# ayutaz/F5-TTS

Measured on AMD Instinct MI355X. Metric: mel-frames/s (RTF alongside), F5TTS_v1_Base NFE=16 CFM.sample, higher is better.
Workload: dtype bf16; 1 GPU; C2: F5TTS_v1_Base CFM.sample, NFE 16 EPSS + sway -1, CFG 2.0, 1 utterance per GPU, 938 prompt + 938 generated frames (1876), 300 tokens; batch_per_gpu=1, frames=1876, gen_frames_per_gpu=938, nfe=16, parallelism=dp1

## Files before the change

f5-tts_amd/csrc/elementwise.hip:

```cpp
#include "common.h"
#include "kernels.h"
#include "lnrow.h"

#include <algorithm>

namespace f5h {

static inline unsigned nblk(int64_t n, int t) { return (unsigned)((n + t - 1) / t); }

struct TVals {
  float t[513];
};
__global__ void time_sinus_kernel(TVals tv, int n, float* out) {
  int i = blockIdx.x * blockDim.x + threadIdx.x;
  if (i >= n * 128) return;
  int r = i / 128, j = i % 128;
  const float k = logf(10000.f) / 127.f;
  float f = expf((float)j * -k);
  float e = (1000.f * tv.t[r]) * f;
  out[r * 256 + j] = sinf(e);
  out[r * 256 + 128 + j] = cosf(e);
}
hipError_t time_sinus(const float* t_host, int n, float* out, hipStream_t st) {
  if (n <= 0 || n > 512) return hipErrorInvalidValue;
// ... 690 lines not shown
  float v = 0.f;
  if (col < 128) {
    if (col < 100 && s < B && !drop_audio && cmask[(int64_t)b * N + n]) v = cond[((int64_t)b * N + n) * 100 + col];
  } else if (col - 128 < td) {
    const float* t = (s < B && !drop_text) ? tc : tu;
    v = t[((int64_t)b * N + n) * td + (col - 128)];
  }
  out[i] = from_f32<TO>(v);
}
hipError_t build_ct(int compute, const float* cond, const uint8_t* cond_mask, const float* text_c,
                    const float* text_u, int B, int N, int td, int S, int drop_audio, int drop_text, void* out,
                    hipStream_t st) {
  const int tdp = (td + 63) / 64 * 64;
  const int64_t total = (int64_t)S * N * (128 + tdp);
  F5H_OP_DISPATCH(compute, T, hipLaunchKernelGGL(build_ct_kernel<T>, dim3(nblk(total, 256)), dim3(256), 0, st, cond, cond_mask, text_c, text_u, B, N, td, tdp, S, drop_audio, drop_text, (T*)out););
  return hipGetLastError();
}

template <typename TO>
__global__ void pack_y_kernel(const float* y, int rows, int mel, TO* yp) {
  int64_t i = (int64_t)blockIdx.x * blockDim.x + threadIdx.x;
  if (i >= (int64_t)rows * 128) return;
  int64_t r = i >> 7;
  int c = (int)(i & 127);
  yp[i] = from_f32<TO>(c < mel ? y[r * mel + c] : 0.f);
}
hipError_t pack_y(int compute, const float* y, int rows, int mel, void* ypad, hipStream_t st) {
  const int64_t total = (int64_t)rows * 128;
  F5H_OP_DISPATCH(compute, T, hipLaunchKernelGGL(pack_y_kernel<T>, dim3(nblk(total, 256)), dim3(256), 0, st, y, rows, mel, (T*)ypad););
  return hipGetLastError();
}

template <typename TO>
__global__ __launch_bounds__(256) void cfg_euler_kernel(EulerArgs a, TO* ypad) {
  int64_t i = (int64_t)blockIdx.x * blockDim.x + threadIdx.x;
  const int64_t total = (int64_t)a.B * a.N * a.mel;
  const int k = a.kstep ? __hip_atomic_load(a.kstep, __ATOMIC_RELAXED, __HIP_MEMORY_SCOPE_AGENT) : 0;
  if (a.kstep && a.next_dst) {
    if (k + 1 < a.nfe) {
      const float4* src = reinterpret_cast<const float4*>(a.next_src + (int64_t)(k + 1) * a.next_stride);
      float4* dst = reinterpret_cast<float4*>(a.next_dst);
      for (int64_t j = i; j < a.next_n / 4; j += (int64_t)gridDim.x * blockDim.x) dst[j] = src[j];
    }
  }
  float dt = a.dt;
  float* traj = a.traj;
  if (a.kstep) {
    dt = sub_nc(a.tgrid[k + 1], a.tgrid[k]);
    traj = a.trajp ? *a.trajp : nullptr;
    if (traj) traj += (int64_t)(k + 1) * total;
  }
  for (; i < total; i += (int64_t)gridDim.x * blockDim.x) {
    const int c = (int)(i % a.mel);
    const int64_t bn = i / a.mel;
    const int b = (int)(bn / a.N), n = (int)(bn - (int64_t)b * a.N);
    const float pc = a.p[(int64_t)b * a.p_seq_stride + (int64_t)(a.p_row_off + n) * a.p_ld + c];
    float v = pc;
    if (a.use_cfg) {
      const float pu = a.p[(int64_t)(a.B + b) * a.p_seq_stride + (int64_t)(a.p_row_off + n) * a.p_ld + c];
      v = add_nc(pc, mul_nc(sub_nc(pc, pu), a.cfg));
    }
    const float y = add_nc(a.y[i], mul_nc(dt, v));
    a.y[i] = y;
    if (ypad) ypad[bn * 128 + c] = from_f32<TO>(y);
    if (traj) traj[i] = y;
  }
  if (a.kstep && a.arrive) {
    __syncthreads();
    if (threadIdx.x == 0) {
      const unsigned old = __hip_atomic_fetch_add(a.arrive, 1u, __ATOMIC_RELAXED, __HIP_MEMORY_SCOPE_AGENT);
      if (old == gridDim.x - 1) {
        __hip_atomic_store(a.arrive, 0u, __ATOMIC_RELAXED, __HIP_MEMORY_SCOPE_AGENT);
        __hip_atomic_store(const_cast<int*>(a.kstep), k + 1, __ATOMIC_RELAXED, __HIP_MEMORY_SCOPE_AGENT);
        if (a.tick) __hip_atomic_fetch_add(a.tick, 1, __ATOMIC_RELAXED, __HIP_MEMORY_SCOPE_AGENT);
      }
    }
  }
}
hipError_t cfg_euler(const EulerArgs& a, hipStream_t st) {
  const int64_t total = (int64_t)a.B * a.N * a.mel;
  const unsigned blocks = std::min<unsigned>(128, std::max<unsigned>(1, nblk(total, 256)));
  F5H_OP_DISPATCH(a.compute, T, hipLaunchKernelGGL(cfg_euler_kernel<T>, dim3(blocks), dim3(256), 0, st, a, (T*)a.ypad););
  return hipGetLastError();
}

template <typename TO, int METHOD>
__global__ __launch_bounds__(256) void cfg_rk_kernel(RkArgs a, TO* ypad) {
  constexpr OdeTableau T = ode_tableau(METHOD);
  constexpr int STAGES = T.stages;
  static_assert(METHOD == 1 || METHOD == 2, "midpoint or rk4");
  static_assert(METHOD != 1 || (T.a[4] == T.c[1] && T.b[0] == 0.f && T.b[1] == 1.f), "midpoint tableau");
  static_assert(METHOD != 2 || (T.a[4] == T.c[1] && T.a[8] == -T.c[1] && T.a[9] == 1.f && T.a[12] == 1.f &&
                                T.a[13] == -1.f && T.a[14] == 1.f && T.b[1] == 3.f * T.b[0] &&
                                T.b[2] == T.b[1] && T.b[3] == T.b[0]),
                "3/8-rule tableau");
  int64_t i = (int64_t)blockIdx.x * blockDim.x + threadIdx.x;
  const int64_t total = (int64_t)a.B * a.N * a.mel;
  const int e = __hip_atomic_load(a.keval, __ATOMIC_RELAXED, __HIP_MEMORY_SCOPE_AGENT);
  const int k = e / STAGES, s = e - k * STAGES;
  if (a.next_dst && e + 1 < a.neval) {
    const float4* src = reinterpret_cast<const float4*>(a.next_src + (int64_t)(e + 1) * a.next_stride);
    float4* dst = reinterpret_cast<float4*>(a.next_dst);
    for (int64_t j = i; j < a.next_n / 4; j += (int64_t)gridDim.x * blockDim.x) dst[j] = src[j];
  }
  const float dt = sub_nc(a.sgrid[k + 1], a.sgrid[k]);
  const bool last = s == STAGES - 1;
  float* traj = (last && a.trajp) ? *a.trajp : nullptr;
  if (traj) traj += (int64_t)(k + 1) * total;
  for (; i < total; i += (int64_t)gridDim.x * blockDim.x) {
    const int c = (int)(i % a.mel);
    const int64_t bn = i / a.mel;
    const int b = (int)(bn / a.N), n = (int)(bn - (int64_t)b * a.N);
    const float pc = a.p[(int64_t)b * a.p_seq_stride + (int64_t)(a.p_row_off + n) * a.p_ld + c];
    float v = pc;
    if (a.use_cfg) {
// ... 221 lines not shown
```

f5-tts_amd/csrc/engine_ctl.cpp:

```cpp
#include "engine_internal.h"
#include "capi_util.h"

thread_local std::string g_err;
int fail(int code, const std::string& msg) {
  g_err = msg;
  return code;
}
int f5h_internal_fail(int code, const std::string& msg) { return fail(code, msg); }

extern "C" {

const char* f5h_last_error(void) { return g_err.c_str(); }
const char* f5h_version(void) { return "f5h 0.1 gfx950"; }

int f5h_probe_enable(f5h_engine* e, int32_t kclass, int32_t enable) {
  if (!e) return fail(F5H_EINVAL, "null engine");
  std::lock_guard<std::mutex> g(e->pm);
  e->probe_class = enable ? kclass : -1;
  if (e->pstamp) {
    HIPCK(hipSetDevice(e->dev));
    HIPCK(hipDeviceSynchronize());
    HIPCK(hipMemset(e->pstamp, 0, 64 * sizeof(unsigned long long)));
    HIPCK(hipMemset(e->pslots, 0xff, (size_t)kProbeEnd * sizeof(unsigned long long)));
    HIPCK(hipMemset(e->pslots + kProbeEnd, 0, (size_t)kProbeEnd * sizeof(unsigned long long)));
// ... 119 lines not shown
    if (e->mx8_count) {
      HIPCK(hipSetDevice(e->dev));
      HIPCK(hipMemcpy(&n, e->mx8_count, sizeof(n), hipMemcpyDeviceToHost));
    }
    *launches = (int64_t)n;
  }
  return 0;
}

int f5h_store_policy_force(int32_t mode) {
  if (mode < -1 || mode > 1) return fail(F5H_EINVAL, "forced store policy must be -1 (off), 0 (plain) or 1 (write-through)");
  store_policy_force(mode);
  g_kernel_epoch.fetch_add(1);
  return 0;
}

int f5h_last_call_host_ms(f5h_engine* e, double* ms, int32_t n) {
  if (!e || !ms || n <= 0) return fail(F5H_EINVAL, "null engine / buffer");
  std::lock_guard<std::mutex> g(e->hm);
  for (int i = 0; i < n; ++i) ms[i] = i < kHostPhases ? e->last_host[i] : 0.0;
  return 0;
}

int f5h_graph_stats(f5h_engine* e, int64_t* captures, int64_t* replays, int32_t* cached) {
  if (!e) return fail(F5H_EINVAL, "null engine");
  std::lock_guard<std::mutex> g(e->gm);
  if (captures) *captures = e->n_captures;
  if (replays) *replays = e->n_replays;
  if (cached) *cached = (int32_t)e->graphs.size();
  return 0;
}

int f5h_gemm_force_config(int32_t cfg) {
  if (cfg != -1 && cfg != 0 && cfg != 1 && cfg != 5 && cfg != 11 && cfg != 12 && cfg != 13)
    return fail(F5H_EINVAL, "gemm config must be -1, 0, 1, 5, 11, 12 or 13");
  gemm_force_config(cfg);
  g_kernel_epoch.fetch_add(1);
  return 0;
}

int f5h_attn_force_safe(int32_t on) {
  attention_force_safe(on);
  g_kernel_epoch.fetch_add(1);
  return 0;
}

}
```

f5-tts_amd/csrc/gemm.hip:

```cpp
#include "gemm_impl.h"

namespace f5h {

static int g_force_cfg = -1;
static int gemm_env_cfg() {
  static int v = [] {
    const char* e = getenv("F5H_GEMM_CFG");
    return e ? atoi(e) : -1;
  }();
  return v;
}


static int large_cfg() {
  static const int v = [] {
    const char* e = getenv("F5H_LARGE_CFG");
    const int c = e ? atoi(e) : 11;
    return (c == 12 || c == 13) ? c : 11;
  }();
  return v;
}

int gemm_group_m() {
  static const int v = [] {
    const char* e = getenv("F5H_GEMM_GROUP_M");
    const int g = e ? atoi(e) : 1;
    return g > 1 && g <= 64 ? g : 1;
  }();
  return v;
}

int gemm_num_cus() {
  static int cus[64] = {0};
  int dev = 0;
  if (hipGetDevice(&dev) != hipSuccess || dev < 0 || dev >= 64) return 256;
  if (!cus[dev]) {
    int n = 0;
    if (hipDeviceGetAttribute(&n, hipDeviceAttributeMultiprocessorCount, dev) != hipSuccess || n <= 0) n = 256;
    cus[dev] = n;
  }
  return cus[dev];
}

static int pick_cfg(const GemmArgs& a) {
  if (a.K % 64 == 0 && (int64_t)((a.M + 255) / 256) * ((a.N + 255) / 256) >= 1024) return large_cfg();
  struct Opt { int cfg, bm, bn; float eff; };
  constexpr Opt opts[3] = {{5, 192, 128, 0.86f}, {1, 128, 128, 0.74f}, {0, 64, 128, 0.57f}};
  int best = 0;
  double tbest = 1e300;
  for (const Opt& o : opts) {
    const int64_t tiles = (int64_t)((a.M + o.bm - 1) / o.bm) * ((a.N + o.bn - 1) / o.bn);
    const double t = (double)((tiles + 511) / 512) * o.bm * o.bn / o.eff;
    if (t < tbest * 0.999) tbest = t, best = o.cfg;
  }
  return best;
}

static int gemm_map_cfg(int N, int K) {
  struct E { int n, k, c; };
  static std::vector<E> m = [] {
    std::vector<E> v;
    const char* e = getenv("F5H_GEMM_MAP");
    while (e && *e) {
      int n, k, c, used = 0;
      if (sscanf(e, "%d:%d:%d%n", &n, &k, &c, &used) != 3) break;
      v.push_back({n, k, c});
      e += used;
      if (*e == ',') ++e;
    }
    return v;
  }();
  for (const E& x : m)
    if (x.n == N && x.k == K) return x.c;
  return -1;
}


int gemm_select_cfg(const GemmArgs& a) {
  int cfg = g_force_cfg >= 0 ? g_force_cfg : gemm_env_cfg();
  if (cfg < 0) cfg = gemm_map_cfg(a.N, a.K);
  if (cfg < 0) cfg = pick_cfg(a);
  return cfg;
}

hipError_t gemm_launch_bf16_a(int epi, const GemmArgs& a, hipStream_t st);
hipError_t gemm_launch_bf16_b(int epi, const GemmArgs& a, hipStream_t st);
hipError_t gemm_launch_f16_a(int epi, const GemmArgs& a, hipStream_t st);
hipError_t gemm_launch_f16_b(int epi, const GemmArgs& a, hipStream_t st);
hipError_t gemm_launch_f32(int epi, const GemmArgs& a, hipStream_t st);

static bool hot_epi(int epi) {
  return epi == EPI_QKV || epi == EPI_RESID || epi == EPI_RESID16 || epi == EPI_GELU_TANH || epi == EPI_GELU_ERF_OP;
}

void gemm_force_config(int cfg) { g_force_cfg = cfg; }

static int g_store_force = -1;
void store_policy_force(int mode) { g_store_force = mode; }
int store_policy_forced() { return g_store_force; }

static bool gemm_wt_variant(int compute, int epi, const GemmArgs& a, int64_t* tiles, int64_t* slots) {
  if (compute == F5H_C_FP32 || (epi != EPI_QKV && epi != EPI_RESID16 && epi != EPI_GELU_TANH) || a.M <= 0) return false;
  const int cfg = gemm_select_cfg(a);
  if (cfg != 0 && cfg != 1 && cfg != 5) return false;
  const int bm = cfg == 0 ? 64 : (cfg == 1 ? 128 : 192);
  *tiles = (int64_t)((a.M + bm - 1) / bm) * ((a.N + 127) / 128);
  *slots = 2 * (int64_t)gemm_num_cus();
  return epi == EPI_QKV ? fast_epi_ok<EPI_QKV>(a, 128)
                        : (epi == EPI_RESID16 ? fast_epi_ok<EPI_RESID16>(a, 128) : fast_epi_ok<EPI_GELU_TANH>(a, 128));
}

int gemm_store_wt(int compute, int epi, const GemmArgs& a, int want) {
  if (g_store_force >= 0) want = g_store_force;
  int64_t tiles = 0, slots = 0;
  if (want == 0 || !gemm_wt_variant(compute, epi, a, &tiles, &slots)) return 0;
  return want > 0 || tiles <= slots;
}

hipError_t gemm(int compute, int epi, const GemmArgs& a0, hipStream_t st) {
  GemmArgs a = a0;
  if (g_store_force >= 0) a.store_wt = gemm_store_wt(compute, epi, a0, g_store_force);
  const int bke = compute ? 64 : 32;
  if (a.K % bke != 0 || a.M < 0 || a.N <= 0 || a.lda % 8 || a.ldw % 8) return hipErrorInvalidValue;
  if (epi == EPI_INPROJ && (a.ldc % 8 || a.ld_add % 8 || a.N % 8)) return hipErrorInvalidValue;
  if (epi == EPI_QKV && (a.N % 64)) return hipErrorInvalidValue;
  if (a.A2 && (a.k_split <= 0 || a.k_split % 64 || a.k_split >= a.K)) return hipErrorInvalidValue;
  if (a.resid && epi != EPI_RESID && epi != EPI_RESID16) return hipErrorInvalidValue;
  switch (compute) {
    case F5H_C_BF16: return hot_epi(epi) ? gemm_launch_bf16_a(epi, a, st) : gemm_launch_bf16_b(epi, a, st);
    case F5H_C_FP16: return hot_epi(epi) ? gemm_launch_f16_a(epi, a, st) : gemm_launch_f16_b(epi, a, st);
    default: return gemm_launch_f32(epi, a, st);
  }
}

}
```

f5-tts_amd/csrc/gemm_impl.h:

```cpp
#pragma once
#include "common.h"
#include "kernels.h"
#include "chain.h"

#include <cstdio>
#include <cstdlib>
#include <vector>

namespace f5h {

int gemm_select_cfg(const GemmArgs& a);


template <int BM, int BN, int WGM, int WGN, int NS, int KB = 128>
struct GemmCfg {
  static constexpr int NW = WGM * WGN, THREADS = 64 * NW;
  static constexpr int WM = BM / WGM, WN = BN / WGN, MT = WM / 16, NT = WN / 16;
  static constexpr int CPR = KB / 16;
  static constexpr int stage_bytes = (BM + BN) * KB;
  static constexpr int main_bytes = NS * stage_bytes;
  static constexpr int EPAD = WN + 4;
  static constexpr int epi_bytes = NW * 16 * EPAD * 4;
  static constexpr int bytes = main_bytes > epi_bytes ? main_bytes : epi_bytes;
  static_assert(KB == 128 || KB == 64, "stage row bytes");
// ... 206 lines not shown
        if (col + e < g.N) C[off + e] = x.v[e];
    }
  }
}

template <int DPS, int X = 0>
F5H_DEV void wait_stages(int n_stages) {
  switch (n_stages) {
    case 0: asm volatile("s_waitcnt vmcnt(%0)" ::"i"(X) : "memory"); break;
    case 1: asm volatile("s_waitcnt vmcnt(%0)" ::"i"(DPS + X) : "memory"); break;
    case 2: asm volatile("s_waitcnt vmcnt(%0)" ::"i"(2 * DPS + X) : "memory"); break;
    case 3: asm volatile("s_waitcnt vmcnt(%0)" ::"i"(3 * DPS + X) : "memory"); break;
    default: asm volatile("s_waitcnt vmcnt(%0)" ::"i"(4 * DPS + X) : "memory"); break;
  }
}

template <int AUX = 0>
F5H_DEV void store16_rs(__amdgpu_buffer_rsrc_t r, uint32_t off, u32x4 v) {
  __builtin_amdgcn_raw_buffer_store_b128(v, r, off, 0, AUX);
}
template <typename TC, int AUX = 0>
F5H_DEV void store8_rs(__amdgpu_buffer_rsrc_t r, uint32_t elem, const V8& x) {
  if constexpr (is16<TC>()) {
    typedef typename Op16<TC>::v8 v8;
    const v8 b = {from_f32<TC>(x.v[0]), from_f32<TC>(x.v[1]), from_f32<TC>(x.v[2]), from_f32<TC>(x.v[3]),
                  from_f32<TC>(x.v[4]), from_f32<TC>(x.v[5]), from_f32<TC>(x.v[6]), from_f32<TC>(x.v[7])};
    store16_rs<AUX>(r, elem * 2u, __builtin_bit_cast(u32x4, b));
  } else {
    store16_rs<AUX>(r, elem * 4u, u32x4{__float_as_uint(x.v[0]), __float_as_uint(x.v[1]), __float_as_uint(x.v[2]),
                                   __float_as_uint(x.v[3])});
    store16_rs<AUX>(r, elem * 4u + 16u, u32x4{__float_as_uint(x.v[4]), __float_as_uint(x.v[5]), __float_as_uint(x.v[6]),
                                         __float_as_uint(x.v[7])});
  }
}

typedef unsigned u32x2_t __attribute__((ext_vector_type(2)));
template <int CTRL>
F5H_DEV float dpp8(float x) {
  return __int_as_float(__builtin_amdgcn_update_dpp(0, __float_as_int(x), CTRL, 0xF, 0xF, false));
}
F5H_DEV float sum8(float v) {
  v = add_nc(v, dpp8<0xB1>(v));
  v = add_nc(v, dpp8<0x4E>(v));
  return add_nc(v, dpp8<0x141>(v));
}
F5H_DEV V8 qk_norm8(V8 x, const V8& w, float eps, bool on) {
  float s = mul_nc(x.v[0], x.v[0]);
#pragma unroll
  for (int e = 1; e < 8; ++e) s = add_nc(s, mul_nc(x.v[e], x.v[e]));
  const float r = rsqrtf(add_nc(mul_nc(sum8(s), 1.f / 64.f), eps));
#pragma unroll
  for (int e = 0; e < 8; ++e) x.v[e] = on ? mul_nc(mul_nc(x.v[e], r), w.v[e]) : x.v[e];
  return x;
}
F5H_DEV float ln_m2_term(float q, float mp, float mean) {
  const float d = sub_nc(mp, mean);
  return __builtin_fmaf(mul_nc(64.f, d), d, q);
}
F5H_DEV float ln_rstd(float m2, float inv_np, float eps) {
  return rsqrtf(__builtin_fmaf(m2, mul_nc(inv_np, 1.f / 64.f), eps));
}
F5H_DEV float sum8_order(const float (&a)[8]) {
  return add_nc(add_nc(add_nc(a[0], a[1]), add_nc(a[2], a[3])), add_nc(add_nc(a[4], a[5]), add_nc(a[6], a[7])));
}
F5H_DEV void ln_row_fetch(const GemmArgs& g, int m0, int tid, int BM, u32x4 (&raw)[8]) {
  const bool on = g.ln_part_in != nullptr;
// ... 36 lines not shown
  const int cc = lane % CH;
  const int col = cbase + cc * 8;
  V8 bias8 = V8{};
  if constexpr (BIAS) bias8 = load8(g.bias + col);
  V8 lnA = V8{}, lnB = V8{};
  __amdgpu_buffer_rsrc_t ln_dst = rsrc_of(nullptr, 0), ln_st = rsrc_of(nullptr, 0);
  int ln_p = 0;
  const int ln_np = g.ln_nparts;
  if constexpr (LNF == 1 || LNF == 4) {
    if constexpr (LNF == 1) {
      lnA = load8(g.hs_scale + col);
#pragma unroll
      for (int e = 0; e < 8; ++e) lnA.v[e] = 1.f + lnA.v[e];
      ln_dst = rsrc_of(g.hs, (uint64_t)g.M * g.ldc * sizeof(TC));
    }
    ln_st = rsrc_of(g.ln_part, (uint64_t)g.M * ln_np * 8);
    ln_p = __builtin_amdgcn_readfirstlane(cbase >> 6);
  } else if constexpr (LNCONS) {
    if (g.ln_u) lnA = load8(g.ln_u + col);
    if (g.ln_v) lnB = load8(g.ln_v + col);
    if constexpr (BIAS) {
#pragma unroll
      for (int e = 0; e < 8; ++e) lnB.v[e] += bias8.v[e];
    }
    if constexpr (LNF == 2) ln_st = rsrc_of(g.ln_part_in, (uint64_t)g.M * ln_np * 8);
  }
  const int lp0 = min(cc, ln_np - 1), lp1 = min(cc + 8, ln_np - 1);
  const float ln_w0 = cc < ln_np ? 1.f : 0.f, ln_w1 = cc + 8 < ln_np ? 1.f : 0.f;
  const float ln_inv_np = 1.f / (float)ln_np;
  V8 gate8 = V8{{1.f, 1.f, 1.f, 1.f, 1.f, 1.f, 1.f, 1.f}};
  if constexpr (EPI == EPI_RESID || EPI == EPI_RESID16)
    if (g.gate) gate8 = load8(g.gate + col);
  int which = 0, head = 0, dh = 0;
  bool rope_on = false;
  float qsc = 1.f;
  __amdgpu_buffer_rsrc_t dst;
  if constexpr (EPI == EPI_QKV) {
    static_assert(WN <= 64 && 64 % WN == 0, "a wave's columns lie in one head");
    const int inner = g.heads * 64;
    which = __builtin_amdgcn_readfirstlane(fdiv(cbase, inner));
    const int hc = col - which * inner;
    head = hc >> 6;
    dh = hc & 63;
    rope_on = which < 2 && head < g.rope_heads;
    qsc = (which == 0 && g.q_scale != 0.f) ? g.q_scale : 1.f;
    dst = rsrc_of(which == 0 ? g.q : (which == 1 ? g.k : g.v), qkv_dst_elems(g, g.qkv_dst_len ? fdiv(g.M, g.seq_len) : 0) * sizeof(TC));
  } else {
    constexpr int OES = (EPI == EPI_STORE || EPI == EPI_RESID || EPI == EPI_INPROJ) ? 4 : (int)sizeof(TC);
    dst = rsrc_of(g.C, (uint64_t)(g.M + (EPI == EPI_INPROJ ? g.dual_rows : 0)) * g.ldc * OES);
  }
  const int dlen = EPI == EPI_QKV ? qkv_panel_rows(g) : 0;
  V8 qkw = V8{};
  if constexpr (QKN) qkw = load8((which == 0 ? g.q_norm_w : g.k_norm_w) + dh);
  const bool qkn_on = which < 2;
  struct RowIn {
    u32x4 d0, d1;
    u32x4 e0, e1;
    uint32_t kb;
    u32x2_t s0, s1;
  };
  const __amdgpu_buffer_rsrc_t rk = rsrc_of(g.rowkeep, g.rowkeep ? (uint64_t)g.M : 0);
  const bool masked = g.rowkeep != nullptr;
  int pf_sq[TPC], pf_pos[TPC], ps_sq[TPC], ps_pos[TPC];
  if constexpr (EPI == EPI_QKV) {
#pragma unroll
    for (int t = 0; t < TPC; ++t) {
      const int row0 = rbase + t * (64 / CH) + lane / CH;
      pf_sq[t] = ps_sq[t] = fdiv(row0, g.seq_len);
      pf_pos[t] = ps_pos[t] = row0 - pf_sq[t] * g.seq_len;
    }
  }
  auto advance = [&](int& sq, int& pos) {
    pos += 16;
    while (pos >= g.seq_len) {
      pos -= g.seq_len;
      ++sq;
    }
  };
  auto fetch = [&](int i, RowIn (&ri)[TPC]) {
#pragma unroll
    for (int t = 0; t < TPC; ++t) {
      const int rr = t * (64 / CH) + lane / CH;
      const int rowc = min(rbase + i * 16 + rr, g.M - 1);
      if constexpr (LNF == 2) {
        ri[t].s0 = __builtin_amdgcn_raw_buffer_load_b64(ln_st, (uint32_t)((rowc * ln_np + lp0) * 8), 0, 0);
        ri[t].s1 = __builtin_amdgcn_raw_buffer_load_b64(ln_st, (uint32_t)((rowc * ln_np + lp1) * 8), 0, 0);
      }
      if constexpr (EPI == EPI_QKV) {
        (void)rowc;
        const u32x4* p = reinterpret_cast<const u32x4*>(g.rope + pf_pos[t] * 32 + (dh >> 1));
        ri[t].d0 = p[0];
        ri[t].d1 = p[1];
        advance(pf_sq[t], pf_pos[t]);
      } else if constexpr (EPI == EPI_RESID || EPI == EPI_RESID16) {
        if constexpr (!PREF) {
          const u32x4* p = reinterpret_cast<const u32x4*>(reinterpret_cast<const ResT<TC, EPI>*>(
                                                              g.resid ? g.resid : g.C) + (int64_t)rowc * g.ldc + col);
          ri[t].d0 = p[0];
          if constexpr (sizeof(ResT<TC, EPI>) == 4) ri[t].d1 = p[1];
        }
        ri[t].kb = __builtin_amdgcn_raw_buffer_load_b8(rk, (uint32_t)rowc, 0, 0);
      } else if constexpr (EPI == EPI_INPROJ) {
        const u32x4* p = reinterpret_cast<const u32x4*>(g.add + (int64_t)rowc * g.ld_add + col);
        ri[t].d0 = p[0];
        ri[t].d1 = p[1];
        const u32x4* p2 = reinterpret_cast<const u32x4*>(g.add + (int64_t)(rowc + g.dual_rows) * g.ld_add + col);
        ri[t].e0 = p2[0];
        ri[t].e1 = p2[1];
      }
    }
  };
  auto as_v8 = [&](const RowIn& ri) -> V8 {
    if constexpr (EPI == EPI_RESID16 && is16<TC>()) {
      typedef typename Op16<TC>::v8 v8;
      const v8 h = __builtin_bit_cast(v8, ri.d0);
      return V8{{to_f32(h[0]), to_f32(h[1]), to_f32(h[2]), to_f32(h[3]), to_f32(h[4]), to_f32(h[5]), to_f32(h[6]),
                 to_f32(h[7])}};
    } else {
      return V8{{__uint_as_float(ri.d0[0]), __uint_as_float(ri.d0[1]), __uint_as_float(ri.d0[2]),
                 __uint_as_float(ri.d0[3]), __uint_as_float(ri.d1[0]), __uint_as_float(ri.d1[1]),
                 __uint_as_float(ri.d1[2]), __uint_as_float(ri.d1[3])}};
    }
  };
  constexpr int RB = PD + 1;
  RowIn rbuf[RB][TPC];
  static_for<0, (PD < MT ? PD : MT)>([&](auto F) { fetch(decltype(F)::value, rbuf[decltype(F)::value % RB]); });
  static_for<0, MT>([&](auto I) {
    constexpr int i = decltype(I)::value;
    if constexpr (i + PD < MT) fetch(i + PD, rbuf[(i + PD) % RB]);
#pragma unroll
    for (int j = 0; j < NT; ++j)
      *reinterpret_cast<f32x4*>(Cs + fr * EPAD + j * 16 + 4 * q) = acc[i][j];
    __builtin_amdgcn_fence(__ATOMIC_RELEASE, "wavefront");
    __builtin_amdgcn_wave_barrier();
    __builtin_amdgcn_fence(__ATOMIC_ACQUIRE, "wavefront");
#pragma unroll
    for (int t = 0; t < TPC; ++t) {
      const int rr = t * (64 / CH) + lane / CH;
      const int row = rbase + i * 16 + rr;
      const float* src = Cs + rr * EPAD + cc * 8;
      const float4 a0 = *reinterpret_cast<const float4*>(src), a1 = *reinterpret_cast<const float4*>(src + 4);
      V8 x{{a0.x, a0.y, a0.z, a0.w, a1.x, a1.y, a1.z, a1.w}};
      const RowIn& ri = rbuf[i % RB][t];
      if constexpr (LNCONS) {
        float m, rstd;
        if constexpr (LNF == 3) {
          const float2 ms = *reinterpret_cast<const float2*>(ln_rows + 2 * (i * 16 + rr));
          m = ms.x;
          rstd = ms.y;
        } else {
        const float m0 = __uint_as_float(ri.s0.x), m1 = __uint_as_float(ri.s1.x);
        m = mul_nc(sum8(add_nc(ln_w0 * m0, ln_w1 * m1)), ln_inv_np);
        const float e0 = ln_m2_term(__uint_as_float(ri.s0.y), m0, m), e1 = ln_m2_term(__uint_as_float(ri.s1.y), m1, m);
        rstd = ln_rstd(sum8(add_nc(ln_w0 * e0, ln_w1 * e1)), ln_inv_np, g.ln_eps);
        }
#pragma unroll
        for (int e = 0; e < 8; e += 2) {
          const f32x2 t = f32x2{x.v[e], x.v[e + 1]} - f32x2{m, m} * f32x2{lnA.v[e], lnA.v[e + 1]};
          const f32x2 y = f32x2{rstd, rstd} * t + f32x2{lnB.v[e], lnB.v[e + 1]};
          x.v[e] = y.x;
          x.v[e + 1] = y.y;
        }
      }
      if constexpr (BIAS && !LNCONS) {
#pragma unroll
        for (int e = 0; e < 8; ++e) x.v[e] = add_nc(x.v[e], bias8.v[e]);
      }
      if constexpr (QKN) x = qk_norm8(x, qkw, g.qk_norm_eps, qkn_on);
      if constexpr (EPI == EPI_QKV) {
        const V8 cs = as_v8(ri);
#pragma unroll
        for (int p = 0; p < 4; ++p) {
          const float c = cs.v[2 * p], sn = cs.v[2 * p + 1];
          const f32x2 ab = {x.v[2 * p], x.v[2 * p + 1]};
          f32x2 r;
          {
#pragma clang fp contract(off)
            const f32x2 pc = ab * c, ps = f32x2{ab.y, ab.x} * sn;
            r = pc + f32x2{-ps.x, ps.y};
            r = (rope_on ? r : ab) * qsc;
          }
          x.v[2 * p] = r.x;
          x.v[2 * p + 1] = r.y;
        }
        (void)row;
        store8_rs<TC, AUX>(dst, (uint32_t)(((ps_sq[t] * g.heads + head) * dlen + ps_pos[t]) * 64 + dh), x);
        advance(ps_sq[t], ps_pos[t]);
      } else if constexpr (EPI == EPI_RESID || EPI == EPI_RESID16) {
        V8 c;
        if constexpr (PREF)
          c = pre[PREF ? i : 0][PREF ? t : 0];
        else
          c = as_v8(ri);
        const bool keep = !masked || ri.kb;
        V8 o;
#pragma unroll
        for (int e = 0; e < 8; ++e) o.v[e] = resid_add(c.v[e], gate8.v[e], x.v[e], keep);
        store8_rs<ResT<TC, EPI>, AUX>(dst, (uint32_t)((int64_t)row * g.ldc + col), o);
        if constexpr (LNF == 1 || LNF == 4) {
          V8 hr, hv;
          f32x2 s2 = {0.f, 0.f};
#pragma unroll
          for (int e = 0; e < 8; e += 2) {
            const f32x2 h2 = {to_f32(from_f32<TC>(o.v[e])), to_f32(from_f32<TC>(o.v[e + 1]))};
            hr.v[e] = h2.x;
            hr.v[e + 1] = h2.y;
            if constexpr (LNF == 1) {
              const f32x2 v2 = h2 * f32x2{lnA.v[e], lnA.v[e + 1]};
              hv.v[e] = v2.x;
              hv.v[e + 1] = v2.y;
              s2 += h2;
            }
          }
          if constexpr (LNF == 1) store8_rs<TC, AUX>(ln_dst, (uint32_t)((int64_t)row * g.ldc + col), hv);
          const float mean = LNF == 4 ? 0.f : sum8(s2.x + s2.y) * (1.f / 64.f);
          f32x2 q2 = {0.f, 0.f};
#pragma unroll
          for (int e = 0; e < 8; e += 2) {
            const f32x2 dv = f32x2{hr.v[e], hr.v[e + 1]} - f32x2{mean, mean};
            q2 += dv * dv;
          }
          const float m2 = sum8(q2.x + q2.y);
          __builtin_amdgcn_raw_buffer_store_b64(u32x2_t{__float_as_uint(mean), __float_as_uint(m2)}, ln_st,
                                                (uint32_t)((row * ln_np + ln_p) * 8), 0, 0);
        }
      } else if constexpr (EPI == EPI_GELU_TANH || EPI == EPI_GELU_ERF_OP) {
        if constexpr (EPI == EPI_GELU_TANH && is16<TC>()) {
#pragma unroll
          for (int e = 0; e < 8; e += 2) {
            const f32x2 gv = gelu_tanh_fast2(f32x2{x.v[e], x.v[e + 1]});
            x.v[e] = gv.x;
            x.v[e + 1] = gv.y;
          }
        } else {
#pragma unroll
          for (int e = 0; e < 8; ++e) x.v[e] = EPI == EPI_GELU_ERF_OP ? gelu_erf(x.v[e]) : gelu_tanh(x.v[e]);
        }
        store8_rs<TC, AUX>(dst, (uint32_t)((int64_t)row * g.ldc + col), x);
      } else if constexpr (EPI == EPI_STORE16) {
        store8_rs<TC, AUX>(dst, (uint32_t)((int64_t)row * g.ldc + col), x);
      } else if constexpr (EPI == EPI_INPROJ) {
        V8 o0, o1;
#pragma unroll
        for (int e = 0; e < 4; ++e) {
          o0.v[e] = x.v[e] + __uint_as_float(ri.d0[e]);
          o0.v[e + 4] = x.v[e + 4] + __uint_as_float(ri.d1[e]);
          o1.v[e] = x.v[e] + __uint_as_float(ri.e0[e]);
          o1.v[e + 4] = x.v[e + 4] + __uint_as_float(ri.e1[e]);
        }
        constexpr uint32_t kPast = 0xF0000000u / 4;
        store8_rs<float, AUX>(dst, row < g.M ? (uint32_t)((int64_t)row * g.ldc + col) : kPast, o0);
        if (g.dual_rows)
          store8_rs<float, AUX>(dst, row < g.M ? (uint32_t)((int64_t)(row + g.dual_rows) * g.ldc + col) : kPast, o1);
      } else {
        store8_rs<float, AUX>(dst, (uint32_t)((int64_t)row * g.ldc + col), x);
      }
    }
    __builtin_amdgcn_fence(__ATOMIC_RELEASE, "wavefront");
    __builtin_amdgcn_wave_barrier();
    __builtin_amdgcn_fence(__ATOMIC_ACQUIRE, "wavefront");
  });
}
template <typename TC, int EPI, int MT, int NT, int WN, int EPAD, bool PREF, int AUX = 0, int PD = 1, bool FOLD = true,
          bool QKN = false, int PM, int PT>
F5H_DEV void epilogue_fast(const GemmArgs& g, const f32x4 (&acc)[MT][NT], float* Cs, int rbase, int cbase,
                           int lane, const V8 (&pre)[PM][PT], const float* ln_rows = nullptr) {
  if constexpr (WN == 64 && is16<TC>() && FOLD) {
    if constexpr (EPI == EPI_RESID16) {
      if (g.ln_part && g.ln_rms) {
        if (g.bias)
          epilogue_fast_t<TC, EPI, MT, NT, WN, EPAD, PREF, true, PM, PT, AUX, PD, 4>(g, acc, Cs, rbase, cbase, lane, pre);
        else
          epilogue_fast_t<TC, EPI, MT, NT, WN, EPAD, PREF, false, PM, PT, AUX, PD, 4>(g, acc, Cs, rbase, cbase, lane, pre);
        return;
      }
      if (g.ln_part) {
        if (g.bias)
          epilogue_fast_t<TC, EPI, MT, NT, WN, EPAD, PREF, true, PM, PT, AUX, PD, 1>(g, acc, Cs, rbase, cbase, lane, pre);
        else
          epilogue_fast_t<TC, EPI, MT, NT, WN, EPAD, PREF, false, PM, PT, AUX, PD, 1>(g, acc, Cs, rbase, cbase, lane, pre);
        return;
      }
    } else if constexpr (EPI == EPI_GELU_TANH || EPI == EPI_QKV) {
      if (g.ln_part_in && ln_rows) {
        if (g.bias)
          epilogue_fast_t<TC, EPI, MT, NT, WN, EPAD, PREF, true, PM, PT, AUX, PD, 3, QKN>(g, acc, Cs, rbase, cbase, lane, pre,
                                                                                   ln_rows);
        else
          epilogue_fast_t<TC, EPI, MT, NT, WN, EPAD, PREF, false, PM, PT, AUX, PD, 3, QKN>(g, acc, Cs, rbase, cbase, lane, pre,
                                                                                    ln_rows);
        return;
      }
      if (g.ln_part_in) {
        if (g.bias)
// ... 1168 lines not shown
  if (a.q_norm_w)
    hipLaunchKernelGGL((gemm_kernel<TC, EPI_QKV, BM, 128, 2, 2, NS, false, 128, 0, true, true>), dim3(tiles), dim3(256), 0,
                       st, a);
  else
    hipLaunchKernelGGL((gemm_kernel<TC, EPI_QKV, BM, 128, 2, 2, NS, false, 128, 0, false, true>), dim3(tiles), dim3(256),
                       0, st, a);
  return hipGetLastError();
}

template <typename TC, int EPI>
static hipError_t launch_t(const GemmArgs& a, hipStream_t st) {
  if (a.M == 0) return hipSuccess;
  if constexpr (EPI == EPI_QKV) {
    if (a.add) {
      const bool qkn = a.q_norm_w || a.k_norm_w;
      if (a.ln_part_in || a.qkv_dst_len <= 0 || a.heads <= 0 || a.N != 3 * a.heads * 64 ||
          (qkn && (!a.q_norm_w || !a.k_norm_w)))
        return hipErrorInvalidValue;
      if constexpr (std::is_same<TC, bf16>::value) return gemm_launch_rq_bf16(a, st);
      else if constexpr (std::is_same<TC, float>::value) return gemm_launch_rq_f32(a, st);
      else return gemm_launch_rq_f16(a, st);
    }
  }
  int cfg = 0;
  if constexpr (is16<TC>()) cfg = gemm_select_cfg(a);
  const bool qkn = a.q_norm_w || a.k_norm_w;
  if (qkn && (EPI != EPI_QKV || !a.q_norm_w || !a.k_norm_w || a.heads <= 0 || a.N != 3 * a.heads * 64))
    return hipErrorInvalidValue;
  if (a.qkv_dst_len) {
    if (EPI != EPI_QKV || a.ln_part_in || a.seq_len <= 0 || a.qkv_dst_len < a.seq_len || a.M % a.seq_len ||
        a.M >= (1 << 24) || a.heads <= 0 || qkv_dst_elems(a, a.M / a.seq_len) * 4 >= 0xF0000000ull)
      return hipErrorInvalidValue;
  }
  const bool strips = a.ln_part || a.ln_part_in || qkn;
  if (strips && (cfg == 12 || cfg == 13)) cfg = 11;
  if (strips && cfg == 11 && (!fast_epi_ok<EPI>(a, 256) || a.K % 64)) cfg = 1;
  if (a.hs || a.ln_part || a.ln_part_in) {
    const bool prod = a.ln_part && EPI == EPI_RESID16 && (a.ln_rms ? !a.hs && !a.hs_scale : a.hs && a.hs_scale);
    const bool cons = a.ln_part_in && (EPI == EPI_GELU_TANH || EPI == EPI_QKV) &&
                      (a.ln_rms ? !a.ln_u && !a.ln_v : a.ln_u && a.ln_v);
    const int bn = cfg == 11 ? 256 : 128;
    if (!is16<TC>() || (a.ln_part && a.ln_part_in) || !(prod || cons) || a.ln_nparts <= 0 || a.ln_nparts > 16 ||
        (cfg != 0 && cfg != 1 && cfg != 5 && cfg != 11) || !fast_epi_ok<EPI>(a, bn) || (a.rowkeep && !a.ln_rms) ||
        a.live_len)
      return hipErrorInvalidValue;
  }
  if constexpr (EPI == EPI_QKV) {
    if (qkn) {
      if (cfg != 0 && cfg != 1 && cfg != 5 && cfg != 11) return hipErrorInvalidValue;
      if constexpr (std::is_same<TC, bf16>::value) return gemm_launch_qkn_bf16(a, cfg, st);
      else if constexpr (std::is_same<TC, float>::value) return gemm_launch_qkn_f32(a, cfg, st);
      else return gemm_launch_qkn_f16(a, cfg, st);
    }
  }
  switch (cfg) {
    case 0: return launch_cfg<TC, EPI, 64, 128, 2, 2, 3>(a, st);
    case 1: return launch_cfg<TC, EPI, 128, 128, 2, 2, 2>(a, st);
    case 5: return launch_cfg<TC, EPI, 192, 128, 2, 2, 2>(a, st);
    default:
      if constexpr (is16<TC>()) {
        if (a.K % 64) return hipErrorInvalidValue;
        if (cfg != 11 && cfg != 12 && cfg != 13) return hipErrorInvalidValue;
        if (cfg == 11)
          launch_pp<TC, EPI, 256, 256, 1, 4, 1, 3>(a, st);
        else if (cfg == 13)
          launch_ppp<TC, EPI, 256, 256, 1, 4, 1, 3>(a, st);
        else
          launch_8p<TC, EPI>(a, st);
        break;
      }
      return hipErrorInvalidValue;
  }
  return hipGetLastError();
}

template <typename TC>
static hipError_t launch_epi(int epi, const GemmArgs& a, hipStream_t st) {
  switch (epi) {
    case EPI_STORE: return launch_t<TC, EPI_STORE>(a, st);
    case EPI_SILU: return launch_t<TC, EPI_SILU>(a, st);
    case EPI_GELU_TANH: return launch_t<TC, EPI_GELU_TANH>(a, st);
    case EPI_GELU_ERF: return launch_t<TC, EPI_GELU_ERF>(a, st);
    case EPI_RESID: return launch_t<TC, EPI_RESID>(a, st);
    case EPI_RESID16: return launch_t<TC, EPI_RESID16>(a, st);
    case EPI_RESID_FILL: return launch_t<TC, EPI_RESID_FILL>(a, st);
    case EPI_INPROJ: return launch_t<TC, EPI_INPROJ>(a, st);
    case EPI_QKV: return launch_t<TC, EPI_QKV>(a, st);
    case EPI_GELU_ERF_OP: return launch_t<TC, EPI_GELU_ERF_OP>(a, st);
    case EPI_STORE16: return launch_t<TC, EPI_STORE16>(a, st);
  }
// ... 6 lines not shown
```

Before: 20220 mel-frames/s.

## Add small-tile GEMM config for narrow outputs and vectorize CFG Euler step

Adds a new GEMM config 2 (32x64 tiles, 6 stages) that the picker selects when N<=128 and the small-tile grid fits within the CU count. This targets narrow projections such as the mel output head, where 64x128 tiles leave most CUs idle. The config is limited to the plain-store epilogue and falls back to config 0 elsewhere. The CFG Euler update kernel now uses float4 loads and stores when alignment allows, runs 512 threads per block, and moves the next-row copy after the main loop (prefetching the first element) to cut scalar memory traffic and overlap the copy.

```diff
diff --git a/f5-tts_amd/csrc/elementwise.hip b/f5-tts_amd/csrc/elementwise.hip
--- a/f5-tts_amd/csrc/elementwise.hip
+++ b/f5-tts_amd/csrc/elementwise.hip
@@ -746,17 +746,28 @@
 }
 
 template <typename TO>
-__global__ __launch_bounds__(256) void cfg_euler_kernel(EulerArgs a, TO* ypad) {
-  int64_t i = (int64_t)blockIdx.x * blockDim.x + threadIdx.x;
+F5H_DEV void store_row4(TO* p, float x, float y, float z, float w) {
+  if constexpr (sizeof(TO) == 4) {
+    *reinterpret_cast<float4*>(p) = make_float4(x, y, z, w);
+  } else {
+    struct alignas(8) Q { TO v[4]; };
+    *reinterpret_cast<Q*>(p) = Q{{from_f32<TO>(x), from_f32<TO>(y), from_f32<TO>(z), from_f32<TO>(w)}};
+  }
+}
+
+template <typename TO, bool V4>
+__global__ __launch_bounds__(512) void cfg_euler_kernel(EulerArgs a, TO* ypad) {
+  const int64_t tid = (int64_t)blockIdx.x * blockDim.x + threadIdx.x, nthr = (int64_t)gridDim.x * blockDim.x;
   const int64_t total = (int64_t)a.B * a.N * a.mel;
   const int k = a.kstep ? __hip_atomic_load(a.kstep, __ATOMIC_RELAXED, __HIP_MEMORY_SCOPE_AGENT) : 0;
-  if (a.kstep && a.next_dst) {
-    if (k + 1 < a.nfe) {
-      const float4* src = reinterpret_cast<const float4*>(a.next_src + (int64_t)(k + 1) * a.next_stride);
-      float4* dst = reinterpret_cast<float4*>(a.next_dst);
-      for (int64_t j = i; j < a.next_n / 4; j += (int64_t)gridDim.x * blockDim.x) dst[j] = src[j];
-    }
-  }
+  const bool copy_row = a.kstep && a.next_dst && k + 1 < a.nfe;
+  const float4* const row_src =
+      copy_row ? reinterpret_cast<const float4*>(a.next_src + (int64_t)(k + 1) * a.next_stride) : nullptr;
+  float4* const row_dst = reinterpret_cast<float4*>(a.next_dst);
+  const int64_t row_n4 = a.next_n / 4;
+  const bool row_first = copy_row && tid < row_n4;
+  float4 row0 = make_float4(0.f, 0.f, 0.f, 0.f);
+  if (row_first) row0 = row_src[tid];
   float dt = a.dt;
   float* traj = a.traj;
   if (a.kstep) {
@@ -764,21 +775,58 @@
     traj = a.trajp ? *a.trajp : nullptr;
     if (traj) traj += (int64_t)(k + 1) * total;
   }
-  for (; i < total; i += (int64_t)gridDim.x * blockDim.x) {
-    const int c = (int)(i % a.mel);
-    const int64_t bn = i / a.mel;
-    const int b = (int)(bn / a.N), n = (int)(bn - (int64_t)b * a.N);
-    const float pc = a.p[(int64_t)b * a.p_seq_stride + (int64_t)(a.p_row_off + n) * a.p_ld + c];
-    float v = pc;
-    if (a.use_cfg) {
-      const float pu = a.p[(int64_t)(a.B + b) * a.p_seq_stride + (int64_t)(a.p_row_off + n) * a.p_ld + c];
-      v = add_nc(pc, mul_nc(sub_nc(pc, pu), a.cfg));
-    }
-    const float y = add_nc(a.y[i], mul_nc(dt, v));
-    a.y[i] = y;
-    if (ypad) ypad[bn * 128 + c] = from_f32<TO>(y);
-    if (traj) traj[i] = y;
-  }
+  if constexpr (V4) {
+    const int m4 = a.mel >> 2;
+    const bool traj4 = (reinterpret_cast<uintptr_t>(traj) & 15) == 0;
+    for (int64_t j = tid; j < total / 4; j += nthr) {
+      const int64_t bn = j / m4;
+      const int c = (int)(j - bn * m4) * 4;
+      const int b = (int)(bn / a.N), n = (int)(bn - (int64_t)b * a.N);
+      const float* pr = a.p + (int64_t)b * a.p_seq_stride + (int64_t)(a.p_row_off + n) * a.p_ld + c;
+      const float4 pc = *reinterpret_cast<const float4*>(pr);
+      float4 v = pc;
+      if (a.use_cfg) {
+        const float4 pu = *reinterpret_cast<const float4*>(pr + (int64_t)a.B * a.p_seq_stride);
+        v.x = add_nc(pc.x, mul_nc(sub_nc(pc.x, pu.x), a.cfg));
+        v.y = add_nc(pc.y, mul_nc(sub_nc(pc.y, pu.y), a.cfg));
+        v.z = add_nc(pc.z, mul_nc(sub_nc(pc.z, pu.z), a.cfg));
+        v.w = add_nc(pc.w, mul_nc(sub_nc(pc.w, pu.w), a.cfg));
+      }
+      float4 y = reinterpret_cast<const float4*>(a.y)[j];
+      y.x = add_nc(y.x, mul_nc(dt, v.x));
+      y.y = add_nc(y.y, mul_nc(dt, v.y));
+      y.z = add_nc(y.z, mul_nc(dt, v.z));
+      y.w = add_nc(y.w, mul_nc(dt, v.w));
+      reinterpret_cast<float4*>(a.y)[j] = y;
+      if (ypad) store_row4<TO>(ypad + bn * 128 + c, y.x, y.y, y.z, y.w);
+      if (traj) {
+        if (traj4) {
+          reinterpret_cast<float4*>(traj)[j] = y;
+        } else {
+          traj[4 * j] = y.x, traj[4 * j + 1] = y.y, traj[4 * j + 2] = y.z, traj[4 * j + 3] = y.w;
+        }
+      }
+    }
+  } else {
+    for (int64_t i = tid; i < total; i += nthr) {
+      const int c = (int)(i % a.mel);
+      const int64_t bn = i / a.mel;
+      const int b = (int)(bn / a.N), n = (int)(bn - (int64_t)b * a.N);
+      const float pc = a.p[(int64_t)b * a.p_seq_stride + (int64_t)(a.p_row_off + n) * a.p_ld + c];
+      float v = pc;
+      if (a.use_cfg) {
+        const float pu = a.p[(int64_t)(a.B + b) * a.p_seq_stride + (int64_t)(a.p_row_off + n) * a.p_ld + c];
+        v = add_nc(pc, mul_nc(sub_nc(pc, pu), a.cfg));
+      }
+      const float y = add_nc(a.y[i], mul_nc(dt, v));
+      a.y[i] = y;
+      if (ypad) ypad[bn * 128 + c] = from_f32<TO>(y);
+      if (traj) traj[i] = y;
+    }
+  }
+  if (row_first) row_dst[tid] = row0;
+  if (copy_row)
+    for (int64_t j = tid + nthr; j < row_n4; j += nthr) row_dst[j] = row_src[j];
   if (a.kstep && a.arrive) {
     __syncthreads();
     if (threadIdx.x == 0) {
@@ -793,8 +841,15 @@
 }
 hipError_t cfg_euler(const EulerArgs& a, hipStream_t st) {
   const int64_t total = (int64_t)a.B * a.N * a.mel;
-  const unsigned blocks = std::min<unsigned>(128, std::max<unsigned>(1, nblk(total, 256)));
-  F5H_OP_DISPATCH(a.compute, T, hipLaunchKernelGGL(cfg_euler_kernel<T>, dim3(blocks), dim3(256), 0, st, a, (T*)a.ypad););
+  auto al16 = [](const void* p) { return (reinterpret_cast<uintptr_t>(p) & 15) == 0; };
+  const bool v4 = a.mel % 4 == 0 && a.p_ld % 4 == 0 && a.p_seq_stride % 4 == 0 && al16(a.y) && al16(a.p) &&
+                  al16(a.ypad) && al16(a.traj);
+  const unsigned blocks = std::min<unsigned>(128, std::max<unsigned>(1, nblk(v4 ? total / 4 : total, 512)));
+  if (v4) {
+    F5H_OP_DISPATCH(a.compute, T, hipLaunchKernelGGL((cfg_euler_kernel<T, true>), dim3(blocks), dim3(512), 0, st, a, (T*)a.ypad););
+  } else {
+    F5H_OP_DISPATCH(a.compute, T, hipLaunchKernelGGL((cfg_euler_kernel<T, false>), dim3(blocks), dim3(512), 0, st, a, (T*)a.ypad););
+  }
   return hipGetLastError();
 }
 
diff --git a/f5-tts_amd/csrc/engine_ctl.cpp b/f5-tts_amd/csrc/engine_ctl.cpp
--- a/f5-tts_amd/csrc/engine_ctl.cpp
+++ b/f5-tts_amd/csrc/engine_ctl.cpp
@@ -175,8 +175,8 @@
 }
 
 int f5h_gemm_force_config(int32_t cfg) {
-  if (cfg != -1 && cfg != 0 && cfg != 1 && cfg != 5 && cfg != 11 && cfg != 12 && cfg != 13)
-    return fail(F5H_EINVAL, "gemm config must be -1, 0, 1, 5, 11, 12 or 13");
+  if (cfg != -1 && cfg != 0 && cfg != 1 && cfg != 2 && cfg != 5 && cfg != 11 && cfg != 12 && cfg != 13)
+    return fail(F5H_EINVAL, "gemm config must be -1, 0, 1, 2, 5, 11, 12 or 13");
   gemm_force_config(cfg);
   g_kernel_epoch.fetch_add(1);
   return 0;
diff --git a/f5-tts_amd/csrc/gemm.hip b/f5-tts_amd/csrc/gemm.hip
--- a/f5-tts_amd/csrc/gemm.hip
+++ b/f5-tts_amd/csrc/gemm.hip
@@ -44,6 +44,7 @@
 
 static int pick_cfg(const GemmArgs& a) {
   if (a.K % 64 == 0 && (int64_t)((a.M + 255) / 256) * ((a.N + 255) / 256) >= 1024) return large_cfg();
+  if (a.N <= 128 && (int64_t)((a.M + 31) / 32) * ((a.N + 63) / 64) <= gemm_num_cus()) return 2;
   struct Opt { int cfg, bm, bn; float eff; };
   constexpr Opt opts[3] = {{5, 192, 128, 0.86f}, {1, 128, 128, 0.74f}, {0, 64, 128, 0.57f}};
   int best = 0;
@@ -101,7 +102,8 @@
 
 static bool gemm_wt_variant(int compute, int epi, const GemmArgs& a, int64_t* tiles, int64_t* slots) {
   if (compute == F5H_C_FP32 || (epi != EPI_QKV && epi != EPI_RESID16 && epi != EPI_GELU_TANH) || a.M <= 0) return false;
-  const int cfg = gemm_select_cfg(a);
+  int cfg = gemm_select_cfg(a);
+  if (cfg == 2) cfg = 0;
   if (cfg != 0 && cfg != 1 && cfg != 5) return false;
   const int bm = cfg == 0 ? 64 : (cfg == 1 ? 128 : 192);
   *tiles = (int64_t)((a.M + bm - 1) / bm) * ((a.N + 127) / 128);
diff --git a/f5-tts_amd/csrc/gemm_impl.h b/f5-tts_amd/csrc/gemm_impl.h
--- a/f5-tts_amd/csrc/gemm_impl.h
+++ b/f5-tts_amd/csrc/gemm_impl.h
@@ -1826,6 +1826,7 @@
         a.M >= (1 << 24) || a.heads <= 0 || qkv_dst_elems(a, a.M / a.seq_len) * 4 >= 0xF0000000ull)
       return hipErrorInvalidValue;
   }
+  if (cfg == 2 && EPI != EPI_STORE) cfg = 0;
   const bool strips = a.ln_part || a.ln_part_in || qkn;
   if (strips && (cfg == 12 || cfg == 13)) cfg = 11;
   if (strips && cfg == 11 && (!fast_epi_ok<EPI>(a, 256) || a.K % 64)) cfg = 1;
@@ -1850,6 +1851,9 @@
   switch (cfg) {
     case 0: return launch_cfg<TC, EPI, 64, 128, 2, 2, 3>(a, st);
     case 1: return launch_cfg<TC, EPI, 128, 128, 2, 2, 2>(a, st);
+    case 2:
+      if constexpr (is16<TC>() && EPI == EPI_STORE) return launch_cfg<TC, EPI, 32, 64, 2, 2, 6>(a, st);
+      return hipErrorInvalidValue;
     case 5: return launch_cfg<TC, EPI, 192, 128, 2, 2, 2>(a, st);
     default:
       if constexpr (is16<TC>()) {
```

Result: no change. 20260 mel-frames/s (median of 4 runs) (+0.2%).

## Specialize GEMM epilogue on rope/scale/mask flags and strength-reduce QKV addressing

Applied to the files above, without the earlier changes.

Wraps the fast epilogue strip loop in a lambda instantiated per runtime-uniform form (rope on/off, q scaling on/off, row mask on/off). Unused rope-table loads, rowkeep byte loads and select logic are dropped on paths that do not need them. The per-row sequence/position division loop is replaced by an incremental offset with a precomputed wrap delta. Rope, bias and residual math now use packed f32x2 ops via inline asm, and the LN path reuses the packed bf16 output. Code size and register pressure grow from the multiple instantiations, and the inline asm may constrain scheduling.

```diff
diff --git a/f5-tts_amd/csrc/gemm_impl.h b/f5-tts_amd/csrc/gemm_impl.h
--- a/f5-tts_amd/csrc/gemm_impl.h
+++ b/f5-tts_amd/csrc/gemm_impl.h
@@ -262,6 +262,25 @@
     store16_rs<AUX>(r, elem * 4u + 16u, u32x4{__float_as_uint(x.v[4]), __float_as_uint(x.v[5]), __float_as_uint(x.v[6]),
                                          __float_as_uint(x.v[7])});
   }
+}
+
+template <typename TC>
+F5H_DEV uint32_t pack2(f32x2 v) {
+  typedef TC v2 __attribute__((ext_vector_type(2)));
+  return __builtin_bit_cast(uint32_t, v2{from_f32<TC>(v.x), from_f32<TC>(v.y)});
+}
+template <typename TC>
+F5H_DEV f32x2 unpack2(uint32_t w) {
+  typedef TC v2 __attribute__((ext_vector_type(2)));
+  const v2 h = __builtin_bit_cast(v2, w);
+  return f32x2{to_f32(h[0]), to_f32(h[1])};
+}
+F5H_DEV f32x2 rope_pair(f32x2 ab, f32x2 cs) {
+  f32x2 pc, ps, r;
+  asm("v_pk_mul_f32 %0, %1, %2 op_sel_hi:[1,0]" : "=v"(pc) : "v"(ab), "v"(cs));
+  asm("v_pk_mul_f32 %0, %1, %2 op_sel:[1,1] op_sel_hi:[0,1]" : "=v"(ps) : "v"(ab), "v"(cs));
+  asm("v_pk_add_f32 %0, %1, %2 neg_lo:[0,1]" : "=v"(r) : "v"(pc), "v"(ps));
+  return r;
 }
 
 typedef unsigned u32x2_t __attribute__((ext_vector_type(2)));
@@ -364,18 +383,13 @@
   if constexpr (EPI == EPI_RESID || EPI == EPI_RESID16)
     if (g.gate) gate8 = load8(g.gate + col);
   int which = 0, head = 0, dh = 0;
-  bool rope_on = false;
-  float qsc = 1.f;
   __amdgpu_buffer_rsrc_t dst;
   if constexpr (EPI == EPI_QKV) {
     static_assert(WN <= 64 && 64 % WN == 0, "a wave's columns lie in one head");
     const int inner = g.heads * 64;
     which = __builtin_amdgcn_readfirstlane(fdiv(cbase, inner));
-    const int hc = col - which * inner;
-    head = hc >> 6;
-    dh = hc & 63;
-    rope_on = which < 2 && head < g.rope_heads;
-    qsc = (which == 0 && g.q_scale != 0.f) ? g.q_scale : 1.f;
+    head = __builtin_amdgcn_readfirstlane((cbase - which * inner) >> 6);
+    dh = col & 63;
     dst = rsrc_of(which == 0 ? g.q : (which == 1 ? g.k : g.v), qkv_dst_elems(g, g.qkv_dst_len ? fdiv(g.M, g.seq_len) : 0) * sizeof(TC));
   } else {
     constexpr int OES = (EPI == EPI_STORE || EPI == EPI_RESID || EPI == EPI_INPROJ) ? 4 : (int)sizeof(TC);
@@ -393,23 +407,33 @@
   };
   const __amdgpu_buffer_rsrc_t rk = rsrc_of(g.rowkeep, g.rowkeep ? (uint64_t)g.M : 0);
   const bool masked = g.rowkeep != nullptr;
-  int pf_sq[TPC], pf_pos[TPC], ps_sq[TPC], ps_pos[TPC];
+  uint32_t w_pos[TPC], w_off[TPC];
+  const int q16 = EPI == EPI_QKV ? __builtin_amdgcn_readfirstlane(fdiv(16, g.seq_len)) : 0;
+  const int r16 = 16 - q16 * g.seq_len;
+  const uint32_t d_stay = (uint32_t)((q16 * g.heads * dlen + r16) * 64);
+  const uint32_t d_wrap = d_stay + (uint32_t)((g.heads * dlen - g.seq_len) * 64);
+  const uint32_t len256 = (uint32_t)g.seq_len * 256u;
   if constexpr (EPI == EPI_QKV) {
 #pragma unroll
     for (int t = 0; t < TPC; ++t) {
       const int row0 = rbase + t * (64 / CH) + lane / CH;
-      pf_sq[t] = ps_sq[t] = fdiv(row0, g.seq_len);
-      pf_pos[t] = ps_pos[t] = row0 - pf_sq[t] * g.seq_len;
-    }
-  }
-  auto advance = [&](int& sq, int& pos) {
-    pos += 16;
-    while (pos >= g.seq_len) {
-      pos -= g.seq_len;
-      ++sq;
-    }
-  };
-  auto fetch = [&](int i, RowIn (&ri)[TPC]) {
+      const int sq = fdiv(row0, g.seq_len);
+      const int pos = row0 - sq * g.seq_len;
+      w_pos[t] = (uint32_t)pos * 256u;
+      w_off[t] = (uint32_t)(((sq * g.heads + head) * dlen + pos) * 64 + dh);
+    }
+  }
+  auto advance = [&](uint32_t& pos, uint32_t& off) {
+    pos += (uint32_t)r16 * 256u;
+    const bool wrap = pos >= len256;
+    pos = wrap ? pos - len256 : pos;
+    off += wrap ? d_wrap : d_stay;
+  };
+  auto strips = [&](auto FORM) __attribute__((always_inline)) {
+  constexpr bool ROT = EPI == EPI_QKV && (decltype(FORM)::value & 1), SCL = EPI == EPI_QKV && (decltype(FORM)::value & 2);
+  constexpr bool MASKED = (EPI == EPI_RESID || EPI == EPI_RESID16) && (decltype(FORM)::value & 1);
+  uint32_t st_off[PD + 1][TPC];
+  auto fetch = [&](int i, RowIn (&ri)[TPC], uint32_t (&so)[TPC]) {
 #pragma unroll
     for (int t = 0; t < TPC; ++t) {
       const int rr = t * (64 / CH) + lane / CH;
@@ -420,10 +444,14 @@
       }
       if constexpr (EPI == EPI_QKV) {
         (void)rowc;
-        const u32x4* p = reinterpret_cast<const u32x4*>(g.rope + pf_pos[t] * 32 + (dh >> 1));
-        ri[t].d0 = p[0];
-        ri[t].d1 = p[1];
-        advance(pf_sq[t], pf_pos[t]);
+        if constexpr (ROT) {
+          const u32x4* p = reinterpret_cast<const u32x4*>(reinterpret_cast<const char*>(g.rope) +
+                                                          (w_pos[t] + (uint32_t)(dh >> 1) * 8u));
+          ri[t].d0 = p[0];
+          ri[t].d1 = p[1];
+        }
+        so[t] = w_off[t];
+        advance(w_pos[t], w_off[t]);
       } else if constexpr (EPI == EPI_RESID || EPI == EPI_RESID16) {
         if constexpr (!PREF) {
           const u32x4* p = reinterpret_cast<const u32x4*>(reinterpret_cast<const ResT<TC, EPI>*>(
@@ -431,7 +459,7 @@
           ri[t].d0 = p[0];
           if constexpr (sizeof(ResT<TC, EPI>) == 4) ri[t].d1 = p[1];
         }
-        ri[t].kb = __builtin_amdgcn_raw_buffer_load_b8(rk, (uint32_t)rowc, 0, 0);
+        if constexpr (MASKED) ri[t].kb = __builtin_amdgcn_raw_buffer_load_b8(rk, (uint32_t)rowc, 0, 0);
       } else if constexpr (EPI == EPI_INPROJ) {
         const u32x4* p = reinterpret_cast<const u32x4*>(g.add + (int64_t)rowc * g.ld_add + col);
         ri[t].d0 = p[0];
@@ -456,10 +484,12 @@
   };
   constexpr int RB = PD + 1;
   RowIn rbuf[RB][TPC];
-  static_for<0, (PD < MT ? PD : MT)>([&](auto F) { fetch(decltype(F)::value, rbuf[decltype(F)::value % RB]); });
+  static_for<0, (PD < MT ? PD : MT)>([&](auto F) {
+    fetch(decltype(F)::value, rbuf[decltype(F)::value % RB], st_off[decltype(F)::value % RB]);
+  });
   static_for<0, MT>([&](auto I) {
     constexpr int i = decltype(I)::value;
-    if constexpr (i + PD < MT) fetch(i + PD, rbuf[(i + PD) % RB]);
+    if constexpr (i + PD < MT) fetch(i + PD, rbuf[(i + PD) % RB], st_off[(i + PD) % RB]);
 #pragma unroll
     for (int j = 0; j < NT; ++j)
       *reinterpret_cast<f32x4*>(Cs + fr * EPAD + j * 16 + 4 * q) = acc[i][j];
@@ -496,45 +526,68 @@
       }
       if constexpr (BIAS && !LNCONS) {
 #pragma unroll
-        for (int e = 0; e < 8; ++e) x.v[e] = add_nc(x.v[e], bias8.v[e]);
+        for (int e = 0; e < 8; e += 2) {
+          const f32x2 xb = f32x2{x.v[e], x.v[e + 1]} + f32x2{bias8.v[e], bias8.v[e + 1]};
+          x.v[e] = xb.x;
+          x.v[e + 1] = xb.y;
+        }
       }
       if constexpr (QKN) x = qk_norm8(x, qkw, g.qk_norm_eps, qkn_on);
       if constexpr (EPI == EPI_QKV) {
-        const V8 cs = as_v8(ri);
-#pragma unroll
-        for (int p = 0; p < 4; ++p) {
-          const float c = cs.v[2 * p], sn = cs.v[2 * p + 1];
-          const f32x2 ab = {x.v[2 * p], x.v[2 * p + 1]};
-          f32x2 r;
-          {
+        if constexpr (ROT || SCL) {
+#pragma unroll
+          for (int p = 0; p < 4; ++p) {
+            f32x2 r = {x.v[2 * p], x.v[2 * p + 1]};
+            if constexpr (ROT) {
+              const u32x4& d = p < 2 ? ri.d0 : ri.d1;
+              r = rope_pair(r, f32x2{__uint_as_float(d[2 * (p & 1)]), __uint_as_float(d[2 * (p & 1) + 1])});
+            }
+            if constexpr (SCL) {
 #pragma clang fp contract(off)
-            const f32x2 pc = ab * c, ps = f32x2{ab.y, ab.x} * sn;
-            r = pc + f32x2{-ps.x, ps.y};
-            r = (rope_on ? r : ab) * qsc;
+              r = r * g.q_scale;
+            }
+            x.v[2 * p] = r.x;
+            x.v[2 * p + 1] = r.y;
           }
-          x.v[2 * p] = r.x;
-          x.v[2 * p + 1] = r.y;
         }
         (void)row;
-        store8_rs<TC, AUX>(dst, (uint32_t)(((ps_sq[t] * g.heads + head) * dlen + ps_pos[t]) * 64 + dh), x);
-        advance(ps_sq[t], ps_pos[t]);
+        store8_rs<TC, AUX>(dst, st_off[i % RB][t], x);
       } else if constexpr (EPI == EPI_RESID || EPI == EPI_RESID16) {
         V8 c;
         if constexpr (PREF)
           c = pre[PREF ? i : 0][PREF ? t : 0];
         else
           c = as_v8(ri);
-        const bool keep = !masked || ri.kb;
-        V8 o;
-#pragma unroll
-        for (int e = 0; e < 8; ++e) o.v[e] = resid_add(c.v[e], gate8.v[e], x.v[e], keep);
-        store8_rs<ResT<TC, EPI>, AUX>(dst, (uint32_t)((int64_t)row * g.ldc + col), o);
+        typedef ResT<TC, EPI> RT;
+        f32x2 o2[4];
+#pragma unroll
+        for (int e = 0; e < 8; e += 2) {
+          const f32x2 c2 = {c.v[e], c.v[e + 1]};
+          {
+#pragma clang fp contract(off)
+            const f32x2 gx = f32x2{gate8.v[e], gate8.v[e + 1]} * f32x2{x.v[e], x.v[e + 1]};
+            o2[e / 2] = c2 + gx;
+          }
+          if constexpr (MASKED) {
+            const bool keep = ri.kb != 0;
+            o2[e / 2] = f32x2{keep ? o2[e / 2].x : c2.x, keep ? o2[e / 2].y : c2.y};
+          }
+        }
+        u32x4 ow = {0u, 0u, 0u, 0u};
+        if constexpr (is16<RT>()) {
+          ow = u32x4{pack2<RT>(o2[0]), pack2<RT>(o2[1]), pack2<RT>(o2[2]), pack2<RT>(o2[3])};
+          store16_rs<AUX>(dst, (uint32_t)((int64_t)row * g.ldc + col) * 2u, ow);
+        } else {
+          store8_rs<RT, AUX>(dst, (uint32_t)((int64_t)row * g.ldc + col),
+                             V8{{o2[0].x, o2[0].y, o2[1].x, o2[1].y, o2[2].x, o2[2].y, o2[3].x, o2[3].y}});
+        }
         if constexpr (LNF == 1 || LNF == 4) {
           V8 hr, hv;
           f32x2 s2 = {0.f, 0.f};
+          asm("" : "+v"(ow[0]), "+v"(ow[1]), "+v"(ow[2]), "+v"(ow[3]));
 #pragma unroll
           for (int e = 0; e < 8; e += 2) {
-            const f32x2 h2 = {to_f32(from_f32<TC>(o.v[e])), to_f32(from_f32<TC>(o.v[e + 1]))};
+            const f32x2 h2 = unpack2<TC>(ow[e / 2]);
             hr.v[e] = h2.x;
             hr.v[e + 1] = h2.y;
             if constexpr (LNF == 1) {
@@ -592,6 +645,30 @@
     __builtin_amdgcn_wave_barrier();
     __builtin_amdgcn_fence(__ATOMIC_ACQUIRE, "wavefront");
   });
+  };
+  typedef std::integral_constant<int, 0> F0;
+  typedef std::integral_constant<int, 1> F1;
+  if constexpr (EPI == EPI_QKV) {
+    const bool rot = which < 2 && head < g.rope_heads, scl = which == 0 && g.q_scale != 0.f;
+    if (rot) {
+      if (scl)
+        strips(std::integral_constant<int, 3>{});
+      else
+        strips(F1{});
+    } else {
+      if (scl)
+        strips(std::integral_constant<int, 2>{});
+      else
+        strips(F0{});
+    }
+  } else if constexpr (EPI == EPI_RESID || EPI == EPI_RESID16) {
+    if (masked)
+      strips(F1{});
+    else
+      strips(F0{});
+  } else {
+    strips(F0{});
+  }
 }
 template <typename TC, int EPI, int MT, int NT, int WN, int EPAD, bool PREF, int AUX = 0, int PD = 1, bool FOLD = true,
           bool QKN = false, int PM, int PT>
```

Result: no change. 20610 mel-frames/s before, 20790 mel-frames/s after, median of 6 (+0.9%).
